# Bob-cheng/DepthModelHardening

Measured on AMD Instinct MI355X. Metric: adv-train images/sec @1024x320, 10-step PGD, bs32, higher is better.
Workload: dtype f32; 1 GPU; Monodepth2 ResNet18 1024x320, 10-step PGD-L_inf attack on 12 scenes, train batch 32/GPU, stereo photometric+SSIM+smoothness loss (md2), Adam; config_index=2, global_batch=32, per_gpu_batch=32, parallelism=dp1, attack_overlap=False, attack_scenes=12, graph_attack=False

## Files before the change

### depthmodelhardening_amd/csrc/stem_conv_fwd.hip

```cpp
#include "common.hpp"

using namespace dmh;

namespace {

typedef float f32x16 __attribute__((ext_vector_type(16)));

constexpr int NT = 256;
constexpr int TR = 4, TC = 32;
constexpr int RH = 2 * TR + 5;
constexpr int RW = 2 * TC + 6;
constexpr int PLANE = RH * RW;
constexpr int NPAIR = 74;

struct PairDesc { int off; int cls; int k0; int k1; };
__host__ __device__ constexpr PairDesc pair_desc(int j) {
    if (j < 63) {
        const int c = j / 21, r = j % 21, ky = r / 3, kx = 2 * (r % 3);
        return {c * PLANE + ky * RW + kx, 0, c * 49 + ky * 7 + kx, c * 49 + ky * 7 + kx + 1};
    }
    if (j < 72) {
        const int q = j - 63, c = q / 3, ky = 2 * (q % 3);
        return {c * PLANE + ky * RW + 6, 1, c * 49 + ky * 7 + 6, c * 49 + (ky + 1) * 7 + 6};
    }
    if (j == 72) return {6 * RW + 6, 2, 0 * 49 + 48, 1 * 49 + 48};
    return {2 * PLANE + 6 * RW + 6, 0, 2 * 49 + 48, -1};
}

struct SArgs {
    const float* x;
    const float* w;
    float* y;
    int B, H, W, Ho, Wo, gx, gy, ntiles;
    float mean, inv_std;
    const int* org;
    int hw, ww;
};

__global__ __launch_bounds__(NT, 2) void stem_conv_fwd_kernel(const SArgs a) {
    __shared__ float tile[3 * PLANE];
    const int tid = threadIdx.x, lane = tid & 63, wv = tid >> 6;
    const int n = lane & 31, h = lane >> 5;

    float wA[NPAIR], wB[NPAIR];
#pragma unroll
    for (int j = 0; j < NPAIR; ++j) {
        const PairDesc d = pair_desc(j);
        const int kk = h ? d.k1 : d.k0;
        wA[j] = kk >= 0 ? a.w[(size_t)n * 147 + kk] : 0.f;
        wB[j] = kk >= 0 ? a.w[(size_t)(n + 32) * 147 + kk] : 0.f;
    }
    const int base = (2 * wv) * RW + 2 * n;
    const float* b0 = tile + base + (h ? 1 : 0);
    const float* b1 = tile + base + (h ? RW : 0);
    const float* b2 = tile + base + (h ? PLANE : 0);

    const size_t HW = (size_t)a.H * a.W, HWo = (size_t)a.hw * a.ww;
    for (int t = blockIdx.x; t < a.ntiles; t += gridDim.x) {
        int q = t;
        const int bxi = q % a.gx;  q /= a.gx;
        const int byi = q % a.gy;
        const int b = q / a.gy;
        const int wy0 = a.org ? a.org[2 * b] : 0, wx0 = a.org ? a.org[2 * b + 1] : 0;
        const int oy0 = wy0 + byi * TR, ox0 = wx0 + bxi * TC;
        const int iy0 = 2 * oy0 - 3, ix0 = 2 * ox0 - 3;
        const float* xb = a.x + (size_t)b * 3 * HW;
        __syncthreads();
        for (int e = tid; e < 3 * PLANE; e += NT) {
            const int c = e / PLANE, rem = e - c * PLANE, r = rem / RW, cc = rem - r * RW;
            const int iy = iy0 + r, ix = ix0 + cc;
            const bool ok = iy >= 0 && iy < a.H && ix >= 0 && ix < a.W;
            const float v = xb[(size_t)c * HW + (size_t)min(max(iy, 0), a.H - 1) * a.W + min(max(ix, 0), a.W - 1)];
            tile[e] = ok ? (v - a.mean) * a.inv_std : 0.f;
        }
        __syncthreads();
        f32x16 accA, accB;
#pragma unroll
        for (int v = 0; v < 16; ++v) accA[v] = accB[v] = 0.f;
#pragma unroll
        for (int j = 0; j < NPAIR; ++j) {
            const PairDesc d = pair_desc(j);
            const float bv = (d.cls == 0 ? b0 : d.cls == 1 ? b1 : b2)[d.off];
            accA = __builtin_amdgcn_mfma_f32_32x32x2f32(wA[j], bv, accA, 0, 0, 0);
            accB = __builtin_amdgcn_mfma_f32_32x32x2f32(wB[j], bv, accB, 0, 0, 0);
        }
        const int oy = oy0 + wv - wy0, ox = ox0 + n - wx0;
        if (oy < a.hw && ox < a.ww) {
            float* yb = a.y + (size_t)b * 64 * HWo + (size_t)oy * a.ww + ox;
#pragma unroll
            for (int v = 0; v < 16; ++v) {
                const int i = 8 * (v >> 2) + 4 * h + (v & 3);
                yb[(size_t)i * HWo] = accA[v];
                yb[(size_t)(i + 32) * HWo] = accB[v];
            }
        }
    }
}

inline long long stem_fwd_tiles(int B, int hw, int ww) {
    return (long long)B * ((ww + TC - 1) / TC) * ((hw + TR - 1) / TR);
}
inline int stem_fwd_workgroups(long long tiles) { return (int)(tiles < 512 ? tiles : 512); }

}

extern "C" {

static int launch_stem_fwd(const float* x, const float* w, const int* org, int B, int H, int W, int hw, int ww, float mean,
                           float std, float* y, void* stream, const char* fn) {
    SArgs a;
    a.x = x;
    a.w = w;
    a.y = y;
    a.B = B;
    a.H = H;
    a.W = W;
    a.Ho = H / 2;
    a.Wo = W / 2;
    a.org = org;
    a.hw = hw;
    a.ww = ww;
    a.gx = (ww + TC - 1) / TC;
    a.gy = (hw + TR - 1) / TR;
    const long long tiles = stem_fwd_tiles(B, hw, ww);
    if (tiles >= (1ll << 31)) return fail(DMH_EINVAL, "%s: grid too large", fn);
    a.ntiles = (int)tiles;
    a.mean = mean;
    a.inv_std = 1.0f / std;
    const int blocks = stem_fwd_workgroups(tiles);
    hipLaunchKernelGGL(stem_conv_fwd_kernel, dim3(blocks), dim3(NT), 0, (hipStream_t)stream, a);
    return check_launch(fn);
}

int dmh_stem_conv_norm_fwd(const float* x, const float* w, int B, int H, int W, float mean, float std, float* y,
                           void* stream) {
    DMH_REQUIRE(x && w && y, "null pointer");
    DMH_REQUIRE(B > 0 && H >= 2 && W >= 2 && (H & 1) == 0 && (W & 1) == 0, "image height and width must be even");
    DMH_REQUIRE(std > 0.f, "std must be positive");
    DMH_REQUIRE((int64_t)B * 64 * (H / 2) * (W / 2) < ((int64_t)1 << 40), "tensor too large");
    return launch_stem_fwd(x, w, nullptr, B, H, W, H / 2, W / 2, mean, std, y, stream, "dmh_stem_conv_norm_fwd");
}

int64_t dmh_stem_conv_norm_fwd_tiles(int B, int H, int W) {
    if (B <= 0 || H < 2 || W < 2 || (H & 1) || (W & 1)) return -1;
    return stem_fwd_tiles(B, H / 2, W / 2);
}

int dmh_stem_conv_norm_fwd_workgroups(int B, int H, int W) {
    const int64_t tiles = dmh_stem_conv_norm_fwd_tiles(B, H, W);
    return tiles < 0 || tiles >= ((int64_t)1 << 31) ? -1 : stem_fwd_workgroups(tiles);
}

int dmh_stem_conv_norm_fwd_win(const float* x, const float* w, const int* org, int B, int H, int W, int hw, int ww, float mean,
                               float std, float* y, void* stream) {
    DMH_REQUIRE(x && w && y && org, "null pointer");
    DMH_REQUIRE(B > 0 && H >= 2 && W >= 2 && (H & 1) == 0 && (W & 1) == 0, "image height and width must be even");
    DMH_REQUIRE(std > 0.f, "std must be positive");
    DMH_REQUIRE(hw >= 1 && ww >= 1 && hw <= H / 2 && ww <= W / 2, "the window must lie inside the H/2 x W/2 output");
    return launch_stem_fwd(x, w, org, B, H, W, hw, ww, mean, std, y, stream, "dmh_stem_conv_norm_fwd_win");
}

}
```

Measured before the change: 407.4 images/s.

## Double-buffer stem conv input tiles via buffer_load to LDS with prefetch

Replaces the synchronous global-to-LDS tile load in the stem conv with direct buffer_load...lds DMA into a double-buffered LDS tile. The next tile is requested before the current tile's MFMA work and normalised in place afterwards, so the input load overlaps compute. Out-of-bounds elements are handled with buffer offsets and an inside bitmask. This adds inline asm and m0 manipulation, doubles LDS use, and adds a 32-bit offset limit on image size. The stem is a small share of a full adversarial training step.

Measured after the change: 409.1 images/s (median of 6 runs). Within noise of the previous version (+0.4%).

```diff
diff --git a/depthmodelhardening_amd/csrc/stem_conv_fwd.hip b/depthmodelhardening_amd/csrc/stem_conv_fwd.hip
--- a/depthmodelhardening_amd/csrc/stem_conv_fwd.hip
+++ b/depthmodelhardening_amd/csrc/stem_conv_fwd.hip
@@ -37,43 +37,85 @@
     int hw, ww;
 };
 
+constexpr int NDMA = (3 * PLANE + 4 * 64 - 1) / (4 * 64);
+constexpr int TILE_F = 4 * NDMA * 64;
+
+__device__ __forceinline__ int lane_now() {
+    int l;
+    asm volatile("v_mbcnt_lo_u32_b32 %0, -1, 0\n\tv_mbcnt_hi_u32_b32 %0, -1, %0" : "=v"(l));
+    return l;
+}
+
+__device__ __forceinline__ int org_at(const int* org, int i) {
+    return org ? ((const __attribute__((address_space(4))) int*)org)[i] : 0;
+}
+
 __global__ __launch_bounds__(NT, 2) void stem_conv_fwd_kernel(const SArgs a) {
-    __shared__ float tile[3 * PLANE];
-    const int tid = threadIdx.x, lane = tid & 63, wv = tid >> 6;
-    const int n = lane & 31, h = lane >> 5;
+    __shared__ float tile[2 * TILE_F];
+    const int wvu = __builtin_amdgcn_readfirstlane((int)threadIdx.x >> 6);
 
     float wA[NPAIR], wB[NPAIR];
 #pragma unroll
     for (int j = 0; j < NPAIR; ++j) {
         const PairDesc d = pair_desc(j);
+        const int n = threadIdx.x & 31, h = threadIdx.x >> 5 & 1;
         const int kk = h ? d.k1 : d.k0;
         wA[j] = kk >= 0 ? a.w[(size_t)n * 147 + kk] : 0.f;
         wB[j] = kk >= 0 ? a.w[(size_t)(n + 32) * 147 + kk] : 0.f;
     }
-    const int base = (2 * wv) * RW + 2 * n;
-    const float* b0 = tile + base + (h ? 1 : 0);
-    const float* b1 = tile + base + (h ? RW : 0);
-    const float* b2 = tile + base + (h ? PLANE : 0);
-
-    const size_t HW = (size_t)a.H * a.W, HWo = (size_t)a.hw * a.ww;
-    for (int t = blockIdx.x; t < a.ntiles; t += gridDim.x) {
+
+    const unsigned lds0 = (unsigned)(uintptr_t)tile;
+    const unsigned img_bytes = (unsigned)(3 * a.H * a.W) * 4u;
+
+    auto request = [&](int t, int buf) -> unsigned {
         int q = t;
         const int bxi = q % a.gx;  q /= a.gx;
         const int byi = q % a.gy;
         const int b = q / a.gy;
-        const int wy0 = a.org ? a.org[2 * b] : 0, wx0 = a.org ? a.org[2 * b + 1] : 0;
-        const int oy0 = wy0 + byi * TR, ox0 = wx0 + bxi * TC;
-        const int iy0 = 2 * oy0 - 3, ix0 = 2 * ox0 - 3;
-        const float* xb = a.x + (size_t)b * 3 * HW;
-        __syncthreads();
-        for (int e = tid; e < 3 * PLANE; e += NT) {
-            const int c = e / PLANE, rem = e - c * PLANE, r = rem / RW, cc = rem - r * RW;
+        const int wy0 = org_at(a.org, 2 * b), wx0 = org_at(a.org, 2 * b + 1);
+        const int iy0 = 2 * (wy0 + byi * TR) - 3, ix0 = 2 * (wx0 + bxi * TC) - 3;
+        const rsrc_t xrs = make_rsrc(a.x + (size_t)b * 3 * a.H * a.W, img_bytes);
+        unsigned inside = 0;
+        const int e0 = 64 * wvu + lane_now();
+#pragma unroll
+        for (int k = 0; k < NDMA; ++k) {
+            const int e = e0 + 4 * 64 * k, c = e / PLANE, rem = e - c * PLANE, r = rem / RW, cc = rem - r * RW;
             const int iy = iy0 + r, ix = ix0 + cc;
-            const bool ok = iy >= 0 && iy < a.H && ix >= 0 && ix < a.W;
-            const float v = xb[(size_t)c * HW + (size_t)min(max(iy, 0), a.H - 1) * a.W + min(max(ix, 0), a.W - 1)];
-            tile[e] = ok ? (v - a.mean) * a.inv_std : 0.f;
-        }
-        __syncthreads();
+            const bool ok = (unsigned)iy < (unsigned)a.H && (unsigned)ix < (unsigned)a.W &&
+                            (k < NDMA - 1 || e < 3 * PLANE);
+            inside |= ok ? (1u << k) : 0u;
+            const unsigned vo = ok ? (unsigned)((c * a.H + iy) * a.W + ix) * 4u : 0xFFFFFFFFu;
+            const unsigned ldst = __builtin_amdgcn_readfirstlane(lds0 + (unsigned)((buf * TILE_F + (4 * k + wvu) * 64) * 4));
+            unsigned keep;
+            asm volatile("s_mov_b32 %0, m0\n\ts_mov_b32 m0, %3\n\ts_nop 0\n\tbuffer_load_dword %1, %2, 0 offen lds\n\ts_mov_b32 m0, %0"
+                         : "=&s"(keep) : "v"(vo), "s"(xrs), "s"(ldst) : "memory");
+        }
+        return inside;
+    };
+    auto normalise = [&](int buf, unsigned inside) {
+        asm volatile("s_waitcnt vmcnt(0)" ::: "memory");
+        float* tb = tile + buf * TILE_F + wvu * 64 + lane_now();
+#pragma unroll
+        for (int k = 0; k < NDMA; ++k) {
+            const float v = tb[4 * k * 64];
+            tb[4 * k * 64] = (inside >> k & 1u) ? (v - a.mean) * a.inv_std : 0.f;
+        }
+    };
+
+    const size_t HWo = (size_t)a.hw * a.ww;
+    int t = blockIdx.x, buf = 0;
+    normalise(0, request(t, 0));
+    __syncthreads();
+    for (;;) {
+        const int tn = t + (int)gridDim.x;
+        const bool more = tn < a.ntiles;
+        unsigned inside_n = 0;
+        if (more) inside_n = request(tn, buf ^ 1);
+        const int ln = lane_now(), n = ln & 31, h = ln >> 5;
+        const float* tl = tile + buf * TILE_F + (2 * wvu) * RW + 2 * n;
+        const float* b0 = tl + (h ? 1 : 0);
+        const float* b1 = tl + (h ? RW : 0);
+        const float* b2 = tl + (h ? PLANE : 0);
         f32x16 accA, accB;
 #pragma unroll
         for (int v = 0; v < 16; ++v) accA[v] = accB[v] = 0.f;
@@ -84,7 +126,12 @@
             accA = __builtin_amdgcn_mfma_f32_32x32x2f32(wA[j], bv, accA, 0, 0, 0);
             accB = __builtin_amdgcn_mfma_f32_32x32x2f32(wB[j], bv, accB, 0, 0, 0);
         }
-        const int oy = oy0 + wv - wy0, ox = ox0 + n - wx0;
+        if (more) normalise(buf ^ 1, inside_n);
+        int q = t;
+        const int bxi = q % a.gx;  q /= a.gx;
+        const int byi = q % a.gy;
+        const int b = q / a.gy;
+        const int oy = byi * TR + wvu, ox = bxi * TC + n;
         if (oy < a.hw && ox < a.ww) {
             float* yb = a.y + (size_t)b * 64 * HWo + (size_t)oy * a.ww + ox;
 #pragma unroll
@@ -94,6 +141,10 @@
                 yb[(size_t)(i + 32) * HWo] = accB[v];
             }
         }
+        if (!more) break;
+        __syncthreads();
+        t = tn;
+        buf ^= 1;
     }
 }
 
@@ -138,6 +189,7 @@
     DMH_REQUIRE(B > 0 && H >= 2 && W >= 2 && (H & 1) == 0 && (W & 1) == 0, "image height and width must be even");
     DMH_REQUIRE(std > 0.f, "std must be positive");
     DMH_REQUIRE((int64_t)B * 64 * (H / 2) * (W / 2) < ((int64_t)1 << 40), "tensor too large");
+    DMH_REQUIRE((int64_t)H * W < ((int64_t)1 << 28), "image too large (32-bit byte offsets inside an image)");
     return launch_stem_fwd(x, w, nullptr, B, H, W, H / 2, W / 2, mean, std, y, stream, "dmh_stem_conv_norm_fwd");
 }
 
@@ -157,6 +209,7 @@
     DMH_REQUIRE(B > 0 && H >= 2 && W >= 2 && (H & 1) == 0 && (W & 1) == 0, "image height and width must be even");
     DMH_REQUIRE(std > 0.f, "std must be positive");
     DMH_REQUIRE(hw >= 1 && ww >= 1 && hw <= H / 2 && ww <= W / 2, "the window must lie inside the H/2 x W/2 output");
+    DMH_REQUIRE((int64_t)H * W < ((int64_t)1 << 28), "image too large (32-bit byte offsets inside an image)");
     return launch_stem_fwd(x, w, org, B, H, W, hw, ww, mean, std, y, stream, "dmh_stem_conv_norm_fwd_win");
 }
 
```
